# Meryx/ComputeRayTracer

Measured on AMD Instinct MI355X. Metric: Mrays/sec (+ HBM GB/s vs peak), 1080p 250k-tri scene, 1/2/4/8 MI355X, higher is better.
Workload: dtype f32; 1 GPU; S2 atrium250k: 253952 triangles + cornell walls/light, 1920x1080, 64 spp per step (BASELINE config 3)

## Files before the change

computeraytracer_amd/csrc/crt_device.h:

```cpp
#pragma once
#include <hip/hip_runtime.h>
#include <stdint.h>

namespace crt {

constexpr uint32_t kNoHit = 0xFFFFFFFFu;
constexpr int kStackDepth = 64;
constexpr uint32_t kNLambda = 301;
constexpr uint32_t kNCie = 471;
constexpr int CRT_NCOUNTERS_DEV = 16;

struct DevScene {
    const float4 *prim;
    const float4 *primD;
    const uint32_t *slot_of_index;
    const float4 *nodes;
    const float4 *nodes4;
    const uint4 *nodes4q;
    const uint4 *nodes8q;
    const float *spectra;
    const float *cie;
    const float4 *lights;
    uint32_t nprim;
    uint32_t npatch;
    int32_t root;
    int32_t root4;
    int32_t root8;
    uint32_t n_nodes4;
    uint32_t nspectra;
    uint32_t nlight;
    float hit_pad;
    uint32_t nf_last[2];
    float inv_nlight;
    uint32_t W, H;
    float qbase[3], qscale[3];
    float cam[12];
};

struct TraceParams {
    DevScene sc;
    uint32_t x0, y0, tw, th;
    uint32_t band, stride, phase;
    uint32_t first_sample, n_samples;
    float4 *accum;
    uchar4 *rgba;
    unsigned long long *counters;
    uint32_t tiles_x, tiles_y;
};

struct AsTiles {
    const uint32_t *active;
    const uint32_t *base;
    float *q;
    uint32_t n_active;
};

struct AsParams {
    const float4 *accum;
    const float *q;
    const uint32_t *counts;
    float *errors;
    uint32_t *flags;
    uint32_t *active;
    uint32_t *n_active;
    uint32_t tw, th, tiles_x, tiles_y;
    uint32_t min_samples, max_samples;
    float threshold;
};


constexpr uint32_t kWfAlive = 1u, kWfDying = 2u, kWfShadow = 4u, kWfSpecular = 8u, kWfInTrans = 16u;
constexpr uint32_t kWfNanRay = 1u << 31;
constexpr uint32_t kWfHasRad = 1u << 30;
constexpr uint32_t kWfListSlot = 0x7FFFFFFFu, kWfListAlsoExt = 0x80000000u;
constexpr uint32_t kWfDepthShift = 8, kWfLambdaShift = 16;
constexpr uint32_t kWfBatchShift = 25;
constexpr uint32_t kWfRing = 32;
constexpr uint32_t kWfSideCap = 65536;
constexpr uint32_t kWfOverflowLevels = 96;

constexpr uint32_t kWfShards = 64;
struct WfShard { uint32_t n[4], cur, n_dead, pad0[26], alive[kWfRing]; };
static_assert(sizeof(WfShard) == 256, "two lines per shard: the list counters and cursor, the per-batch counts");
struct WfWork { uint32_t cur, pad[31]; };
struct WfCtl {
    WfShard shard[4][kWfShards];
    unsigned long long counters[kWfShards][CRT_NCOUNTERS_DEV];
    uint32_t side_count[kWfRing];
    uint32_t dropped;
};
struct WfWorkQ {
    WfWork work[kWfShards];
    uint32_t work_done;
    uint32_t work_per_shard;
    unsigned long long work_total;
    uint32_t pad_[28];
};
static_assert(sizeof(WfWorkQ) == (kWfShards + 1) * 128, "whole lines");
struct WfSeg {
    unsigned long long work_total;
    uint32_t work_per_shard;
    uint32_t first_sample;
};

struct WfStatus {
    uint32_t it_end;
    uint32_t dropped;
    uint32_t bound;
    uint32_t pad_;
    unsigned long long rays;
    unsigned long long consumed[kWfRing];
    uint32_t left[kWfRing];
    uint32_t alive[kWfRing];
};

constexpr uint32_t kWfFinishSegs = 32;
struct WfFinishSegs {
    struct WfCtl *ctl[kWfFinishSegs];
    uint32_t base[kWfFinishSegs], batch[kWfFinishSegs];
    uint32_t n, blocks_per_seg;
};

struct WfParams {
    DevScene sc;
    float4 *ray_o, *ray_d, *sh_d, *beta, *radiance, *nee;
    uint4 *rng, *misc;
    float2 *hit;
    uint32_t *vis;
    float4 *recA, *recB;
    uint4 *recC;
    uint32_t *dead;
    uint32_t rearm;
    uint32_t gen_blocks;
    float4 *staging[kWfRing];
    uint32_t batch_id;
    WfStatus *status_out;
    uint32_t count_alive;
    uint32_t keep_pool;
    uint32_t side_base[kWfRing];
    uint32_t evict_mask;
    WfCtl *ctl;
    WfWorkQ *wq;
    WfSeg seg[kWfRing];
    uint32_t seg_order[kWfRing];
    uint32_t seg_n;
    uint32_t slot_base;
    uint32_t reset_wq;
    uint32_t P;
    uint32_t x0, y0, tw, th;
    uint32_t band, stride, phase;
    uint32_t tiles_x, tiles_y;
    uint32_t npix_padded;
    uint32_t list_cap;
    uint32_t tail_bound;
    uint32_t n_samples;
    float4 *accum;
    uchar4 *rgba;
    uchar4 *frames;
    uint32_t frame_ring;
    const uint32_t *tea;
    uint32_t count;
    uint32_t trace_form;
    int *stack_overflow;
    uint32_t overflow_lanes;
};

}
```

computeraytracer_amd/csrc/crt_wavefront.hip:

```cpp
#include "crt_shade.h"
#include <algorithm>

namespace crt {

#ifndef CRT_WF_STACK
#define CRT_WF_STACK 32
#endif
#ifndef CRT_WF_REFILL
#define CRT_WF_REFILL 24
#endif
#ifndef CRT_WF_INNER_RUN
#define CRT_WF_INNER_RUN 6
#endif
#ifndef CRT_WF_BURSTS
#define CRT_WF_BURSTS 4
#endif
#ifndef CRT_WF_BVH4
#define CRT_WF_BVH4 1
#endif
#ifndef CRT_WF_LEAF_AT
#define CRT_WF_LEAF_AT 32
#endif
#ifndef CRT_WF_SPEC
#define CRT_WF_SPEC 1
#endif
#ifndef CRT_WF_PATCH_RECOMPUTE
#define CRT_WF_PATCH_RECOMPUTE 20
#endif
#ifndef CRT_WF_SHADE_BLOCK
#define CRT_WF_SHADE_BLOCK 64
#endif
#ifndef CRT_WF_SHADE_MIN_WAVES
#define CRT_WF_SHADE_MIN_WAVES 1
#endif
#ifndef CRT_WF_MIN_WAVES
#define CRT_WF_MIN_WAVES 1
#endif
constexpr int kWfStack = CRT_WF_STACK;
constexpr int kNoNode = 0x7FFFFFFF;
constexpr int kTraceChunk = 128;
constexpr int kRefillAt = CRT_WF_REFILL;

__device__ __forceinline__ uint32_t lane_id() { return threadIdx.x & 63u; }

#ifndef CRT_WF_NT
#define CRT_WF_NT 1
#endif
typedef float v4f __attribute__((ext_vector_type(4)));
typedef float v2f __attribute__((ext_vector_type(2)));
typedef uint32_t v4u __attribute__((ext_vector_type(4)));
#if CRT_WF_NT
__device__ __forceinline__ float4 ldnt(const float4 *p) { const v4f v = __builtin_nontemporal_load((const v4f *)p); return float4{v.x, v.y, v.z, v.w}; }
__device__ __forceinline__ uint4 ldnt(const uint4 *p) { const v4u v = __builtin_nontemporal_load((const v4u *)p); return uint4{v.x, v.y, v.z, v.w}; }
__device__ __forceinline__ float2 ldnt(const float2 *p) { const v2f v = __builtin_nontemporal_load((const v2f *)p); return float2{v.x, v.y}; }
__device__ __forceinline__ uint32_t ldnt(const uint32_t *p) { return __builtin_nontemporal_load(p); }
__device__ __forceinline__ void stnt(float4 *p, float4 v) { __builtin_nontemporal_store(v4f{v.x, v.y, v.z, v.w}, (v4f *)p); }
__device__ __forceinline__ void stnt(uint4 *p, uint4 v) { __builtin_nontemporal_store(v4u{v.x, v.y, v.z, v.w}, (v4u *)p); }
__device__ __forceinline__ void stnt(float2 *p, float2 v) { __builtin_nontemporal_store(v2f{v.x, v.y}, (v2f *)p); }
__device__ __forceinline__ void stnt(uint32_t *p, uint32_t v) { __builtin_nontemporal_store(v, p); }
typedef uint32_t v2u __attribute__((ext_vector_type(2)));
__device__ __forceinline__ void stnt(uint2 *p, uint2 v) { __builtin_nontemporal_store(v2u{v.x, v.y}, (v2u *)p); }
#else
template <class T> __device__ __forceinline__ T ldnt(const T *p) { return *p; }
template <class T> __device__ __forceinline__ void stnt(T *p, T v) { *p = v; }
#endif
__device__ __forceinline__ uint32_t prefix_popc(unsigned long long mask, uint32_t lane)
{
    return (uint32_t)__popcll(mask & ((1ull << lane) - 1ull));
}

__device__ __noinline__ float2 resolve_nonfinite(const float4 *prim, const float4 *primD, const uint32_t *slot_of_index,
                                                 uint32_t nprim, float hit_pad, float ox, float oy, float oz, float dx,
                                                 float dy, float dz, uint32_t exclude)
{
    DevScene S{};
    S.prim = prim; S.primD = primD; S.slot_of_index = slot_of_index; S.nprim = nprim; S.hit_pad = hit_pad;
    float tm = CRT_INFINITY;
    uint32_t bi = kNoHit, bs = kNoHit;
    const f3 o = f3{ox, oy, oz}, d = f3{dx, dy, dz};
    for (uint32_t i = 0; i < nprim; i++) hit_test<true>(S, slot_of_index[i], o, d, exclude, 0.001f, tm, bi, bs);
    return float2{tm, bits_f(bs)};
}

struct PathRegs {
    f3 ray_o, ray_d;
    f4 beta, radiance;
    Rng rng;
    float last_pdf, etaScale;
    uint32_t exclude, work, flags;
};

__device__ __forceinline__ void wavelengths_of(uint32_t lambda, uint32_t wl[4])
{
    wl[0] = lambda; wl[1] = (lambda + 4u) % kNLambda; wl[2] = (lambda + 8u) % kNLambda;
    wl[3] = (lambda + 12u) % kNLambda;
}

struct LightRec { float4 L0, L1, L2, A, B, C, D; uint32_t slot; float pdf_area; };

template <bool UNIFORM>
__device__ __forceinline__ LightRec load_light(const DevScene &S, uint32_t li)
{
    LightRec r;
    r.A = float4{0.0f, 0.0f, 0.0f, 0.0f}; r.B = r.A; r.C = r.A; r.D = r.A; r.slot = kNoHit; r.pdf_area = 0.0f;
    if (UNIFORM) {
        typedef const __attribute__((address_space(4))) v4f *cptr4;
        typedef const __attribute__((address_space(4))) uint32_t *cptr1;
        auto ld = [](cptr4 p) { const v4f v = *p; return float4{v.x, v.y, v.z, v.w}; };
        const cptr4 lg = (cptr4)S.lights;
        r.L0 = ld(lg); r.L1 = ld(lg + 1); r.L2 = ld(lg + 2);
        const uint32_t include = f_bits(r.L1.w);
        if (include < S.nprim) {
            r.slot = ((cptr1)S.slot_of_index)[include];
            const cptr4 pg = (cptr4)S.prim + 3 * (size_t)r.slot;
            r.A = ld(pg); r.B = ld(pg + 1); r.C = ld(pg + 2); r.D = ld((cptr4)S.primD + r.slot);
            r.pdf_area = r.L2.w;
        }
    } else {
        r.L0 = S.lights[3 * li + 0]; r.L1 = S.lights[3 * li + 1]; r.L2 = S.lights[3 * li + 2];
        const uint32_t include = f_bits(r.L1.w);
        if (include < S.nprim) {
            r.slot = S.slot_of_index[include];
            r.A = S.prim[3 * (size_t)r.slot + 0]; r.B = S.prim[3 * (size_t)r.slot + 1]; r.C = S.prim[3 * (size_t)r.slot + 2];
            r.D = S.primD[r.slot];
            uint32_t l2 = (f_bits(r.A.w) >> 4) & 0x3FFFu;
            if (l2 >= S.nlight) l2 = S.nlight - 1u;
            r.pdf_area = S.lights[3 * l2 + 2].w;
        }
    }
    return r;
}

__device__ __forceinline__ f4 nee_term(const DevScene &S, const LightRec &L, f3 pos, f3 ldir, float t_l, float cos_theta,
                                       const f4 spec)
{
    f3 lp, ln; uint32_t lmeta;
    hit_attributes_rec(L.A, L.B, L.C, L.D, pos, ldir, t_l, lp, ln, lmeta);
    f4 le = spec * cos_theta;
    float pdf_l = compute_light_pdf_area(L.pdf_area, S.inv_nlight, lp, ln, pos, ldir);
    float pdf_b = cos_theta / CRT_PI;
    float weight_l = power_heuristic(1.0f, pdf_l, 1.0f, pdf_b);
    return (le * weight_l) / pdf_l;
}

struct ShadeCnt { uint32_t rays = 0, bounces = 0, shadow = 0, hits = 0, paths = 0, prims = 0, walk = 0; };
struct ShadowOut { bool emit; f3 d; float t_l; uint32_t l_index, l_slot; };

template <bool COUNT, bool FINISH>
__device__ __forceinline__ ShadowOut light_sample(const WfParams &P, const LightRec &L, uint32_t slot, f3 pos, f3 nrm, uint32_t b_index,
                                                  float u, float v2, f4 brdf, f4 beta, f4 &radiance, bool &rad_dirty, const uint32_t wl[4], ShadeCnt &cn)
{
    const DevScene &S = P.sc;
    ShadowOut out{false, f3{0.0f, 0.0f, 0.0f}, 0.0f, 0u, 0u};
    f3 pl = (xyz(L.L0) + xyz(L.L1) * u) + xyz(L.L2) * v2;
    f3 ldir = normalize(pl - pos);
    const uint32_t include = f_bits(L.L1.w);
    if (COUNT) { cn.rays++; cn.shadow++; }
    float t_l = CRT_INFINITY;
    uint32_t l_index = kNoHit, l_slot = kNoHit;
    const bool sh_finite = finite3(ldir) && finite3(pos);
    if (include < S.nprim && sh_finite) {
        hit_test_rec<false>(L.A, L.B, L.C, L.D, S.hit_pad, L.slot, pos, ldir, b_index, 0.001f, t_l, l_index, l_slot);
        if (COUNT) cn.prims++;
    }
    const float cos_theta = max_(0.0f, dot(nrm, ldir));
    if (!sh_finite) {
        const uint32_t w = S.nf_last[0] != b_index ? S.nf_last[0] : S.nf_last[1];
        if (COUNT) cn.prims += S.nprim;
        if (w != kNoHit && w == include) {
            if (COUNT) cn.hits++;
            const float qn = bits_f(0x7FC00000u);
            radiance = radiance + f4{qn, qn, qn, qn};
            rad_dirty = true;
        }
    } else if (l_slot != kNoHit && cos_theta > 0.0f) {
        if (COUNT) cn.hits++;
        const f4 nee = nee_term(S, L, pos, ldir, t_l, cos_theta, sample_spectrum(S, f_bits(L.L0.w), wl));
        f4 c = (brdf * nee) * beta;
#ifndef CRT_WHATIF_NO_NEE
        stnt(&P.nee[slot], float4{c.x, c.y, c.z, c.w});
#else
        if (c.x == 12345.678f) stnt(&P.nee[slot], float4{c.x, c.y, c.z, c.w});
#endif
        if (FINISH) {
            P.sh_d[slot] = float4{ldir.x, ldir.y, ldir.z, t_l};
            P.vis[slot] = include;
        }
        out = ShadowOut{true, ldir, t_l, include, l_slot};
        if (COUNT) cn.walk++;
    }
    return out;
}

struct ShadeOut {
    bool alive, emit_ext, emit_sh, sh_primary, rad_dirty; uint32_t batch;
    PathRegs R;
    f3 sd; float t_l; uint32_t l_index, l_slot;
};

#ifdef CRT_WF_PROBE
#define CRT_PROBE(tp, k) if (tp) { asm volatile("s_waitcnt vmcnt(0) lgkmcnt(0)" ::: "memory"); (tp)[k] = __builtin_readcyclecounter(); }
#else
#define CRT_PROBE(tp, k)
#endif

template <bool COUNT, bool FINISH>
__device__ __forceinline__ ShadeOut shade_body(const WfParams &P, uint32_t slot, bool in_pool, ShadeCnt &cn, unsigned long long *tp = nullptr)
{
    const DevScene &S = P.sc;
    PathRegs R;
    R.flags = 0;
    LightRec LU{};
    if (S.nlight == 1u) LU = load_light<true>(S, 0u);
    uint4 misc = uint4{0, 0, 0, 0}, rs = uint4{0, 0, 0, 0};
    float4 v_ro = float4{0, 0, 0, 0}, v_rd = v_ro, v_beta = v_ro, v_rad = v_ro, v_nee = v_ro;
    float2 h = float2{0.0f, 0.0f};
    uint32_t vis_in = 0;
    if (in_pool) {
        misc = ldnt(&P.misc[slot]); v_ro = ldnt(&P.ray_o[slot]); v_rd = ldnt(&P.ray_d[slot]); v_beta = ldnt(&P.beta[slot]);
        v_rad = ldnt(&P.radiance[slot]); rs = ldnt(&P.rng[slot]); h = ldnt(&P.hit[slot]); vis_in = ldnt(&P.vis[slot]);
#ifndef CRT_WHATIF_NO_NEE
        v_nee = ldnt(&P.nee[slot]);
#endif
    }
    CRT_PROBE(tp, 1)
    R.work = misc.x; R.flags = misc.y; R.last_pdf = bits_f(misc.z); R.etaScale = bits_f(misc.w);
    bool alive = in_pool && (R.flags & kWfAlive);
    bool emit_ext = false, emit_sh = false;
    bool sh_primary = false;
    bool finished = false, rad_dirty = false;
    f3 out_sd = f3{0, 0, 0}; float out_tl = 0.0f; uint32_t out_lindex = 0, out_lslot = 0;
    const bool nan_ray = alive && (R.flags & kWfNanRay) != 0u;
    if (nan_ray) R.flags &= ~kWfNanRay;
    const uint32_t h_slot = f_bits(h.y);
    const bool has_hit = alive && !nan_ray && !(R.flags & kWfDying) && h_slot != kNoHit;
    float4 hA = float4{0, 0, 0, 0}, hB = hA, hC = hA, hD = hA;
    if (has_hit) { hA = S.prim[3 * (size_t)h_slot + 0]; hB = S.prim[3 * (size_t)h_slot + 1]; hC = S.prim[3 * (size_t)h_slot + 2]; if (S.npatch) hD = S.primD[h_slot]; }
    CRT_PROBE(tp, 2)

    if (alive) {
        R.ray_o = xyz(v_ro); R.exclude = f_bits(v_ro.w);
        R.ray_d = xyz(v_rd);
        R.beta = f4{v_beta.x, v_beta.y, v_beta.z, v_beta.w};
        R.radiance = (R.flags & kWfHasRad) ? f4{v_rad.x, v_rad.y, v_rad.z, v_rad.w} : f4{0.0f, 0.0f, 0.0f, 0.0f};
        R.rng = Rng{rs.x, rs.y, rs.z, rs.w};
        uint32_t wl[4];
        wavelengths_of((R.flags >> kWfLambdaShift) & 0x1FFu, wl);
        uint32_t depth = (R.flags >> kWfDepthShift) & 0xFFu;

        if (R.flags & kWfShadow) {
            if (vis_in == 1u) { R.radiance = R.radiance + f4{v_nee.x, v_nee.y, v_nee.z, v_nee.w}; rad_dirty = true; }
            R.flags &= ~kWfShadow;
        }
        if (R.flags & kWfDying) {
            finished = true;
        } else if (nan_ray) {
            emit_ext = true;
        } else {
            const uint32_t b_slot = h_slot;
            if (COUNT) cn.bounces++;
            if (b_slot == kNoHit) {
                finished = true;
            } else {
                f3 pos, nrm;
                const f3 o = R.ray_o, d = R.ray_d;
                const uint32_t meta = f_bits(hA.w);
                pos = ray_at(o, d, h.x);
                if ((meta & 3u) == 1u) {
                    nrm = normalize(pos - xyz(hA));
                } else {
                    const f3 n0 = ((meta & 3u) == 0u) ? xyz(hD) : normalize(cross(xyz(hB), xyz(hC)));
                    nrm = (dot(n0, d) > 0.0f) ? -n0 : n0;
                }
                if (COUNT) cn.hits++;
                const uint32_t b_index = f_bits(hB.w);
                R.exclude = b_index;
                const uint32_t material = (meta >> 2) & 3u;
                const uint32_t emission_index = (meta >> 4) & 0x3FFFu;
                const uint32_t reflectance_index = (meta >> 18) & 0x3FFFu;
                if (material == kLight) {
                    f4 le = sample_spectrum(S, emission_index, wl);
                    if (depth == 0 || (R.flags & kWfSpecular)) {
                        R.radiance = R.radiance + R.beta * le;
                    } else {
                        float pdf_l = compute_light_pdf(S, emission_index, pos, nrm, o, d);
                        float weight_b = power_heuristic(1.0f, R.last_pdf, 1.0f, pdf_l);
                        R.radiance = R.radiance + (le * weight_b) * R.beta;
                    }
                    finished = true;
                } else if (depth >= kMaxDepthPath) {
                    finished = true;
                } else {
                    if (R.flags & kWfInTrans) {
                        float distance = length(o - pos);
                        f4 ext = sample_spectrum(S, S.nspectra - 1u, wl);
                        f4 att = f4{exp_(-ext.x * distance), exp_(-ext.y * distance), exp_(-ext.z * distance),
                                    exp_(-ext.w * distance)};
                        R.beta = R.beta * att;
                    }
                    if (material == kDiffuse) {
                        f4 brdf = sample_spectrum(S, reflectance_index, wl) / CRT_PI;
                        float u0 = rnd(R.rng);
                        uint32_t li = (uint32_t)((float)S.nlight * u0);
                        if (li >= S.nlight) li = S.nlight - 1u;
                        float u = rnd(R.rng);
                        float v2 = rnd(R.rng);
                        ShadowOut sh;
                        if (S.nlight == 1u) sh = light_sample<COUNT, FINISH>(P, LU, slot, pos, nrm, b_index, u, v2, brdf, R.beta, R.radiance, rad_dirty, wl, cn);
                        else sh = light_sample<COUNT, FINISH>(P, load_light<false>(S, li), slot, pos, nrm, b_index, u, v2, brdf, R.beta, R.radiance, rad_dirty, wl, cn);
                        if (sh.emit) {
                            emit_sh = true;
                            sh_primary = depth == 0u;
                            R.flags |= kWfShadow;
                            out_sd = sh.d; out_tl = sh.t_l; out_lindex = sh.l_index; out_lslot = sh.l_slot;
                        }
                        f3 new_direction = cosine_hemisphere(R.rng, nrm, R.last_pdf);
                        float cos_theta2 = abs_(dot(nrm, new_direction));
                        R.beta = R.beta * ((brdf * cos_theta2) / R.last_pdf);
                        R.ray_o = pos;
                        R.ray_d = new_direction;
                        R.flags &= ~kWfSpecular;
                    } else if (material == kGlass) {
                        const float eta1 = 1.0f, eta2 = 1.5f;
                        float eta = eta1 / eta2;
                        float cos_theta = dot(nrm, d);
                        float reflected = fresnel_s(d, nrm, eta1, eta2);
                        float pr = reflected;
                        float pt = 1.0f - reflected;
                        float u = rnd(R.rng);
                        f3 current_normal = nrm;
                        if (cos_theta > 0.0f) { eta = 1.0f / eta; current_normal = -current_normal; }
                        f3 new_direction;
                        if (u < pr / (pr + pt)) {
                            new_direction = reflect_(d, current_normal);
                        } else {
                            new_direction = normalize(refract_(d, current_normal, eta));
                            R.beta = R.beta * (eta * eta);
                            R.etaScale = R.etaScale / (eta * eta);
                            R.flags ^= kWfInTrans;
                        }
                        R.ray_o = pos;
                        R.flags |= kWfSpecular;
                        R.exclude = 0xFFFFFFFFu;
                        R.ray_d = new_direction;
                    }
                    bool rr_break = false;
                    {
                        f4 rbeta = R.beta * R.etaScale;
                        float max_beta_component = max_(rbeta.x, max_(rbeta.y, rbeta.z));
                        if (depth > 1u && max_beta_component < 1.0f) {
                            float qq = max_(0.0f, 1.0f - max_beta_component);
                            if (rnd(R.rng) < qq) rr_break = true;
                            else R.beta = R.beta / (1.0f - qq);
                        }
                    }
                    if (rr_break) {
                        if (emit_sh) R.flags |= kWfDying;
                        else finished = true;
                    } else {
                        depth++;
                        R.flags = (R.flags & ~(0xFFu << kWfDepthShift)) | (depth << kWfDepthShift);
                        emit_ext = true;
                        if (COUNT) { cn.rays++; cn.walk++; }
                    }
                }
            }
        }
        if (finished) {
            const uint32_t sample_off = R.work / P.npix_padded, pp = R.work % P.npix_padded;
            const uint32_t tile = pp >> 6, l = pp & 63u;
            const uint32_t lx = (tile % P.tiles_x) * 8u + (l & 7u), ly = (tile / P.tiles_x) * 8u + (l >> 3);
            f3 c = spectral_to_xyz(S, R.radiance, wl);
            stnt(&P.staging[(R.flags >> kWfBatchShift) & (kWfRing - 1u)][(size_t)sample_off * ((size_t)P.tw * P.th) + (size_t)ly * P.tw + lx], float4{c.x, c.y, c.z, 0.0f});
            alive = false;
            if (COUNT) cn.paths++;
        }
    }

    CRT_PROBE(tp, 3)
    if (!alive) R.flags = 0;
    ShadeOut so;
    so.alive = alive; so.emit_ext = emit_ext; so.emit_sh = emit_sh; so.sh_primary = sh_primary; so.rad_dirty = rad_dirty;
    so.batch = (R.flags >> kWfBatchShift) & (kWfRing - 1u);
    so.R = R; so.sd = out_sd; so.t_l = out_tl; so.l_index = out_lindex; so.l_slot = out_lslot;
    return so;
}

template <bool COUNT, bool FINISH>
__device__ __forceinline__ uint32_t shade_store(const WfParams &P, uint32_t slot, bool in_pool, ShadeOut &so, ShadeCnt &cn)
{
    const DevScene &S = P.sc;
    PathRegs &R = so.R;
    uint32_t resolved = 0u;
    if (in_pool) {
        const float4 vo = so.alive ? float4{R.ray_o.x, R.ray_o.y, R.ray_o.z, bits_f(R.exclude)} : float4{S.cam[9], S.cam[10], S.cam[11], bits_f(0xFFFFFFFFu)};
        stnt(&P.ray_o[slot], vo);
        if (so.alive) {
            if (so.emit_ext && (!finite3(R.ray_o) || !finite3(R.ray_d))) {
                P.hit[slot] = resolve_nonfinite(S.prim, S.primD, S.slot_of_index, S.nprim, S.hit_pad, R.ray_o.x, R.ray_o.y, R.ray_o.z,
                                                R.ray_d.x, R.ray_d.y, R.ray_d.z, R.exclude);
                if (COUNT) cn.prims += S.nprim;
                resolved = 1u;
            }
            stnt(&P.ray_d[slot], float4{R.ray_d.x, R.ray_d.y, R.ray_d.z, bits_f(resolved)});
            if (so.rad_dirty || (FINISH && !(R.flags & kWfHasRad))) {
                stnt(&P.radiance[slot], float4{R.radiance.x, R.radiance.y, R.radiance.z, R.radiance.w});
                R.flags |= kWfHasRad;
            }
            stnt(&P.rng[slot], uint4{R.rng.x, R.rng.y, R.rng.z, R.rng.w});
#ifdef CRT_WHATIF_EXTRA_STREAM
            if (!FINISH) { const float4 x = ldnt(&P.sh_d[slot]); stnt(&P.sh_d[slot], float4{x.y, x.x, x.w, x.z}); }
#endif
        }
        stnt(&P.beta[slot], so.alive ? float4{R.beta.x, R.beta.y, R.beta.z, R.beta.w} : float4{1.0f, 1.0f, 1.0f, 1.0f});
        stnt(&P.misc[slot], so.alive ? uint4{R.work, R.flags, f_bits(R.last_pdf), f_bits(R.etaScale)} : uint4{0u, 0u, f_bits(1.0f), f_bits(1.0f)});
    }
    return resolved;
}

__device__ __noinline__ void write_status(const WfCtl *ctl, const WfWorkQ *wq, uint32_t it_end, WfStatus *out)
{
    const uint32_t lane = lane_id();
    const WfShard &sh = ctl->shard[(it_end - 1u) & 3u][lane];
    const uint32_t mine = sh.n[0] + sh.n[1] + sh.n[2] + sh.n[3];
    unsigned long long rays = mine;
    uint32_t bound = mine;
    for (int off = 32; off > 0; off >>= 1) {
        rays += __shfl_xor(rays, off, 64);
        bound = max(bound, (uint32_t)__shfl_xor((int)bound, off, 64));
    }
    if (lane == 0) { out->dropped = ctl->dropped; out->bound = bound; out->pad_ = 0; out->rays = rays; }
#pragma unroll 1
    for (uint32_t g = 0; g < kWfRing; g += 8u) {
        unsigned long long cur[8];
        uint32_t alive[8];
#pragma unroll
        for (uint32_t k = 0; k < 8u; k++) {
            cur[k] = __hip_atomic_load(&wq[g + k].work[lane].cur, __ATOMIC_RELAXED, __HIP_MEMORY_SCOPE_AGENT);
            alive[k] = sh.alive[g + k];
        }
#pragma unroll
        for (uint32_t k = 0; k < 8u; k++) {
            const uint32_t b = g + k;
            const uint32_t wps = wq[b].work_per_shard;
            const unsigned long long wtot = wq[b].work_total, lo = (unsigned long long)lane * wps;
            const unsigned long long size = lo < wtot ? min((unsigned long long)wps, wtot - lo) : 0ull;
            unsigned long long cons = min(cur[k], size);
            const unsigned long long left = __ballot(cur[k] < size);
            uint32_t al = alive[k];
            for (int off = 32; off > 0; off >>= 1) {
                al += (uint32_t)__shfl_xor((int)al, off, 64);
                cons += __shfl_xor(cons, off, 64);
            }
            if (lane == 0) { out->alive[b] = al; out->consumed[b] = cons; out->left[b] = left ? 1u : 0u; }
        }
    }
    if (lane == 0) {
        __threadfence_system();
        __hip_atomic_store(&out->it_end, it_end, __ATOMIC_RELEASE, __HIP_MEMORY_SCOPE_SYSTEM);
    }
}

template <bool COUNT>
__global__ __launch_bounds__(CRT_WF_SHADE_BLOCK, CRT_WF_SHADE_MIN_WAVES) void k_wf_shade(const WfParams P, uint32_t it)
{
    const uint32_t ring = it & 3u, lbuf = it & 1u;
    WfCtl *ctl = P.ctl;
    static_assert(kWfShards == 64, "one lane per shard");
    if (blockIdx.x == 0 && threadIdx.x < 64u && P.status_out != nullptr) write_status(P.ctl, P.wq, it, P.status_out);
    if (blockIdx.x == 0 && threadIdx.x < kWfShards) {
        WfShard &nx = ctl->shard[(it + 1u) & 3u][threadIdx.x];
        nx.n[0] = 0; nx.n[1] = 0; nx.n[2] = 0; nx.n[3] = 0; nx.cur = 0; nx.n_dead = 0;
        for (uint32_t b = 0; b < kWfRing; b++) nx.alive[b] = 0;
    }
    uint32_t slot, my_shard;
    bool in_pool;
    if (P.tail_bound == 0u) {
        const uint32_t local = blockIdx.x * (uint32_t)CRT_WF_SHADE_BLOCK + threadIdx.x;
        slot = P.slot_base + local;
        my_shard = blockIdx.x % kWfShards;
        in_pool = local < P.P;
    } else {
        const uint32_t bps = (4u * P.tail_bound + (uint32_t)CRT_WF_SHADE_BLOCK - 1u) / (uint32_t)CRT_WF_SHADE_BLOCK;
        my_shard = blockIdx.x / bps;
        const uint32_t j = (blockIdx.x % bps) * (uint32_t)CRT_WF_SHADE_BLOCK + threadIdx.x;
        const WfShard &pv = ctl->shard[(it + 3u) & 3u][my_shard];
        const size_t region = (size_t)my_shard * P.list_cap;
        slot = 0; in_pool = false;
        const uint32_t cls = j / P.tail_bound, e = j % P.tail_bound;
        if (cls < 4u && e < pv.n[cls]) {
            const size_t g = (size_t)((lbuf ^ 1u) * 4u + cls) * ((size_t)P.list_cap * kWfShards) + region + e;
            const uint32_t entry = cls < 2u ? f_bits(ldnt(&P.recB[g]).w) : ldnt(&P.recC[g]).x;
            slot = entry & kWfListSlot;
            in_pool = cls < 2u || !(entry & kWfListAlsoExt);
        }
    }
    if (P.evict_mask) {
        uint4 misc = uint4{0, 0, 0, 0};
        if (in_pool) misc = P.misc[slot];
        const uint32_t par = (misc.y >> kWfBatchShift) & (kWfRing - 1u);
        const bool go = in_pool && (misc.y & kWfAlive) && ((P.evict_mask >> par) & 1u);
        for (uint32_t b = 0; b < kWfRing; b++) {
            if (!((P.evict_mask >> b) & 1u)) continue;
            const unsigned long long m = __ballot(go && par == b);
            if (!m) continue;
            uint32_t base = 0;
            if (lane_id() == 0) base = atomicAdd(&ctl->side_count[b], (uint32_t)__popcll(m));
            base = __shfl(base, 0, 64);
            const uint32_t idx = base + prefix_popc(m, lane_id());
            if (go && par == b && idx >= kWfSideCap) atomicAdd(&ctl->dropped, 1u);
            if (go && par == b && idx < kWfSideCap) {
                const uint32_t d = P.side_base[b] + idx;
                P.ray_o[d] = P.ray_o[slot]; P.ray_d[d] = P.ray_d[slot]; P.sh_d[d] = P.sh_d[slot]; P.beta[d] = P.beta[slot];
                P.radiance[d] = P.radiance[slot]; P.nee[d] = P.nee[slot]; P.rng[d] = P.rng[slot]; P.hit[d] = P.hit[slot];
                P.vis[d] = P.vis[slot]; P.misc[d] = misc;
                P.misc[slot] = uint4{0, 0, 0, 0};
            }
        }
    }
    ShadeCnt cn;
#ifdef CRT_WF_PROBE
    unsigned long long tpa[8];
    unsigned long long *tp = (!COUNT && P.tail_bound == 0u && (blockIdx.x & 255u) == 7u) ? tpa : nullptr;
    tpa[0] = __builtin_readcyclecounter();
#else
    unsigned long long *tp = nullptr;
#endif
    ShadeOut so = shade_body<COUNT, false>(P, slot, in_pool, cn, tp);
    CRT_PROBE(tp, 4)
    const bool emit_ext = so.emit_ext, emit_sh = so.emit_sh, sh_primary = so.sh_primary;
    {
        const uint32_t lane = lane_id();
        const bool cl2 = emit_sh && sh_primary, cl3 = emit_sh && !sh_primary;
        const bool dead = in_pool && !so.alive && P.rearm != 0u;
        const unsigned long long m1 = __ballot(emit_ext), m2 = __ballot(cl2), m3 = __ballot(cl3), md = __ballot(dead);
        WfShard &sh = ctl->shard[ring][my_shard];
        uint32_t b1 = 0, b2 = 0, b3 = 0, bd = 0;
        if (lane == 0) {
            if (m1) b1 = atomicAdd(&sh.n[1], (uint32_t)__popcll(m1));
            if (m2) b2 = atomicAdd(&sh.n[2], (uint32_t)__popcll(m2));
            if (m3) b3 = atomicAdd(&sh.n[3], (uint32_t)__popcll(m3));
            if (md) bd = atomicAdd(&sh.n_dead, (uint32_t)__popcll(md));
        }
        if (P.count_alive) {
            unsigned long long am = __ballot(so.alive);
            while (am) {
                const uint32_t b = (uint32_t)__shfl((int)so.batch, __ffsll((long long)am) - 1, 64);
                const unsigned long long m = __ballot(so.alive && so.batch == b);
                if (lane == 0) atomicAdd(&sh.alive[b], (uint32_t)__popcll(m));
                am &= ~m;
            }
        }
        const uint32_t resolved = shade_store<COUNT, false>(P, slot, in_pool, so, cn);
        CRT_PROBE(tp, 5)
        b1 = __shfl(b1, 0, 64); b2 = __shfl(b2, 0, 64); b3 = __shfl(b3, 0, 64); bd = __shfl(bd, 0, 64);
        const size_t region = (size_t)my_shard * P.list_cap;
        const size_t cls_stride = (size_t)P.list_cap * kWfShards;
        const PathRegs &R = so.R;
        if (emit_ext) {
            const size_t g = (size_t)(lbuf * 4u + 1u) * cls_stride + region + b1 + prefix_popc(m1, lane);
            stnt(&P.recA[g], float4{R.ray_o.x, R.ray_o.y, R.ray_o.z, bits_f(R.exclude)});
            stnt(&P.recB[g], float4{R.ray_d.x, R.ray_d.y, R.ray_d.z, bits_f(slot | (resolved ? kWfListAlsoExt : 0u))});
        }
        if (emit_sh) {
            const uint32_t c = cl2 ? 2u : 3u;
            const size_t g = (size_t)(lbuf * 4u + c) * cls_stride + region + (cl2 ? b2 + prefix_popc(m2, lane) : b3 + prefix_popc(m3, lane));
            stnt(&P.recA[g], float4{R.ray_o.x, R.ray_o.y, R.ray_o.z, bits_f(R.exclude)});
            stnt(&P.recB[g], float4{so.sd.x, so.sd.y, so.sd.z, so.t_l});
            stnt(&P.recC[g], uint4{slot | (emit_ext ? kWfListAlsoExt : 0u), so.l_index, so.l_slot, 0u});
        }
        if (dead) stnt(&P.dead[region + bd + prefix_popc(md, lane)], slot);
    }
    if (COUNT) {
        wave_add(ctl->counters[blockIdx.x % kWfShards] + CRT_CNT_RAYS, cn.rays);
        wave_add(ctl->counters[blockIdx.x % kWfShards] + CRT_CNT_BOUNCES, cn.bounces);
        wave_add(ctl->counters[blockIdx.x % kWfShards] + CRT_CNT_SHADOW, cn.shadow);
        wave_add(ctl->counters[blockIdx.x % kWfShards] + CRT_CNT_HITS, cn.hits);
        wave_add(ctl->counters[blockIdx.x % kWfShards] + CRT_CNT_PATHS, cn.paths);
        wave_add(ctl->counters[blockIdx.x % kWfShards] + CRT_CNT_PRIMS, cn.prims);
        wave_add(ctl->counters[blockIdx.x % kWfShards] + CRT_CNT_WALKED, cn.walk);
    }
#ifdef CRT_WF_PROBE
    CRT_PROBE(tp, 6)
    if (tp && lane_id() == 0) {
        for (int k = 0; k < 6; k++) atomicAdd(ctl->counters[blockIdx.x % kWfShards] + 8 + k, tp[k + 1] - tp[k]);
        atomicAdd(ctl->counters[blockIdx.x % kWfShards] + 14, 1ull);
    }
#endif
}

__device__ __forceinline__ uint32_t wf_as_tile(const AsTiles &A, uint32_t w)
{
    return A.active[(w % (A.n_active * 64u)) >> 6];
}

template <bool COUNT, bool ADAPT>
__global__ __launch_bounds__(64) void k_wf_gen(const WfParams P, uint32_t it, const AsTiles A)
{
    const DevScene &S = P.sc;
    const uint32_t ring = it & 3u, lbuf = it & 1u;
    WfCtl *ctl = P.ctl;
    const uint32_t lane = lane_id();
    const uint32_t my_shard = blockIdx.x % kWfShards, j = blockIdx.x / kWfShards;
    WfShard &sh = ctl->shard[ring][my_shard];
    const uint32_t n_chunks = min(sh.n_dead, P.list_cap) / 64u;
    if (j >= n_chunks) return;
    const uint32_t mine = (n_chunks - j + P.gen_blocks - 1u) / P.gen_blocks;
    const size_t region = (size_t)my_shard * P.list_cap;
    const size_t cls_stride = (size_t)P.list_cap * kWfShards;
    uint32_t seg_q[2] = {0, 0}, seg_n[2] = {0, 0}, nseg = 0, want = mine;
    uint32_t seg_w[2] = {0, 0};
    for (uint32_t si = 0; si < P.seg_n && want > 0u && nseg < 2u; si++) {
        const uint32_t sg = P.seg_order[si];
        WfWorkQ *wq = P.wq + sg;
        const uint32_t wps = P.seg[sg].work_per_shard;
        const unsigned long long wtot = P.seg[sg].work_total, lo = (unsigned long long)my_shard * wps;
        const uint32_t size = lo < wtot ? (uint32_t)min((unsigned long long)wps, wtot - lo) : 0u;
        if (__hip_atomic_load(&wq->work[my_shard].cur, __ATOMIC_RELAXED, __HIP_MEMORY_SCOPE_AGENT) >= size) continue;
        uint32_t base = 0;
        if (lane == 0) base = atomicAdd(&wq->work[my_shard].cur, want * 64u);
        base = (uint32_t)__builtin_amdgcn_readfirstlane((int)base);
        if (base >= size) continue;
        const uint32_t got = min(want, (size - base) / 64u);
        seg_q[nseg] = sg; seg_w[nseg] = (uint32_t)lo + base; seg_n[nseg] = got; nseg++;
        want -= got;
    }
    for (uint32_t si = 0; si < P.seg_n && nseg == 0u; si++) {
        const uint32_t sg = P.seg_order[si];
        WfWorkQ *wq = P.wq + sg;
        if (__hip_atomic_load(&wq->work_done, __ATOMIC_RELAXED, __HIP_MEMORY_SCOPE_AGENT) != 0u) continue;
        const uint32_t wps = P.seg[sg].work_per_shard;
        const unsigned long long wtot = P.seg[sg].work_total, lo_l = (unsigned long long)lane * wps;
        const uint32_t size_l = lo_l < wtot ? (uint32_t)min((unsigned long long)wps, wtot - lo_l) : 0u;
        const uint32_t cur_l = __hip_atomic_load(&wq->work[lane].cur, __ATOMIC_RELAXED, __HIP_MEMORY_SCOPE_AGENT);
        const unsigned long long avail = __ballot(cur_l < size_l);
        if (!avail) {
            if (lane == 0) __hip_atomic_store(&wq->work_done, 1u, __ATOMIC_RELAXED, __HIP_MEMORY_SCOPE_AGENT);
            continue;
        }
        const uint32_t rot = my_shard & 63u;
        const unsigned long long rmask = rot ? ((avail >> rot) | (avail << (64u - rot))) : avail;
        const uint32_t s_pick = ((uint32_t)(__ffsll((long long)rmask) - 1) + rot) & 63u;
        uint32_t base = 0;
        if (lane == 0) base = atomicAdd(&wq->work[s_pick].cur, want * 64u);
        base = (uint32_t)__builtin_amdgcn_readfirstlane((int)base);
        const uint32_t size_s = (uint32_t)__shfl((int)size_l, (int)s_pick, 64);
        if (base >= size_s) continue;
        const uint32_t got = min(want, (size_s - base) / 64u);
        seg_q[0] = sg; seg_w[0] = s_pick * wps + base; seg_n[0] = got; nseg = 1;
        want -= got;
    }
    const uint32_t total = seg_n[0] + seg_n[1];
    if (total == 0u) return;
    const bool ragged = ((P.tw | P.th) & 7u) != 0u;
    uint32_t n_valid[2] = {seg_n[0] * 64u, seg_n[1] * 64u};
    if (ragged) {
        for (uint32_t g = 0; g < 2u; g++) {
            n_valid[g] = 0;
            for (uint32_t k = 0; k < seg_n[g]; k++) {
                const uint32_t tile = ADAPT ? wf_as_tile(A, seg_w[g] + 64u * k) : ((seg_w[g] + 64u * k) % P.npix_padded) >> 6;
                const uint32_t lx = (tile % P.tiles_x) * 8u + (lane & 7u), ly = (tile / P.tiles_x) * 8u + (lane >> 3);
                n_valid[g] += (uint32_t)__popcll(__ballot(lx < P.tw && ly < P.th));
            }
        }
    }
    uint32_t b0 = 0;
    if (lane == 0) {
        b0 = atomicAdd(&sh.n[0], n_valid[0] + n_valid[1]);
        if (P.count_alive) {
            if (n_valid[0]) atomicAdd(&sh.alive[seg_q[0]], n_valid[0]);
            if (n_valid[1]) atomicAdd(&sh.alive[seg_q[1]], n_valid[1]);
        }
    }
    uint32_t c_rays = 0, pos = 0;
    bool have_b0 = false;
    for (uint32_t k = 0; k < total; k++) {
        const uint32_t g = k < seg_n[0] ? 0u : 1u, kk = g ? k - seg_n[0] : k;
        const uint32_t sg = seg_q[g];
        const uint32_t w0 = seg_w[g] + 64u * kk;
        uint32_t sample_off = w0 / P.npix_padded, pp0 = w0 % P.npix_padded;
        if (ADAPT) {
            sample_off = w0 / (A.n_active * 64u);
            pp0 = wf_as_tile(A, w0) * 64u;
        }
        const uint32_t tile = pp0 >> 6;
        const uint32_t lx = (tile % P.tiles_x) * 8u + (lane & 7u), ly = (tile / P.tiles_x) * 8u + (lane >> 3);
        const bool valid = lx < P.tw && ly < P.th;
        const unsigned long long mv = __ballot(valid);
        const uint32_t slot = ldnt(&P.dead[region + (size_t)(j + k * P.gen_blocks) * 64u + lane]);
        f3 eye = f3{0.0f, 0.0f, 0.0f}, d = eye;
        uint32_t resolved = 0u;
        if (valid) {
            const uint32_t px = P.x0 + lx, sample = ADAPT ? A.base[tile] + P.seg[sg].first_sample + sample_off : P.seg[sg].first_sample + sample_off;
            const uint32_t py = P.y0 + (ly / P.band) * P.band * P.stride + P.phase * P.band + ly % P.band;
            Rng rng = Rng{py, px * 100u, sample, P.tea[(size_t)ly * P.tw + lx]};
            const float jx = rnd(rng);
            const float fs = ((float)px + ((float)(sample % kGrid) + jx) / (float)kGrid) / (float)S.W;
            const float jy = rnd(rng);
            const float ft = ((float)S.H - (float)py + ((float)(sample % kGrid) + jy) / (float)kGrid) / (float)S.H;
            const f3 llc = f3{S.cam[0], S.cam[1], S.cam[2]}, hor = f3{S.cam[3], S.cam[4], S.cam[5]};
            const f3 ver = f3{S.cam[6], S.cam[7], S.cam[8]};
            eye = f3{S.cam[9], S.cam[10], S.cam[11]};
            d = normalize(((llc + hor * fs) + ver * ft) - eye);
            const float ul = rnd(rng);
            const uint32_t lambda = (uint32_t)(301.0f * ul);
            const bool nan_ray = !finite3(eye) || !finite3(d);
            const uint32_t flags = kWfAlive | (lambda << kWfLambdaShift) | (sg << kWfBatchShift) | (nan_ray ? kWfNanRay : 0u);
            stnt(&P.ray_d[slot], float4{d.x, d.y, d.z, bits_f(0u)});
            stnt(&P.rng[slot], uint4{rng.x, rng.y, rng.z, rng.w});
            stnt((uint2 *)&P.misc[slot], uint2{(ADAPT ? sample_off * P.npix_padded + pp0 : w0) + lane, flags});
            if (!finite3(eye) || !finite3(d)) resolved = 1u;
        }
        if (!have_b0) { b0 = (uint32_t)__builtin_amdgcn_readfirstlane((int)b0); have_b0 = true; }
        if (valid) {
            const size_t e = (size_t)(lbuf * 4u) * cls_stride + region + b0 + pos + prefix_popc(mv, lane);
            stnt(&P.recA[e], float4{eye.x, eye.y, eye.z, bits_f(0xFFFFFFFFu)});
            stnt(&P.recB[e], float4{d.x, d.y, d.z, bits_f(slot | (resolved ? kWfListAlsoExt : 0u))});
            if (COUNT) c_rays++;
        }
        pos += (uint32_t)__popcll(mv);
    }
    if (COUNT) {
        wave_add(ctl->counters[blockIdx.x % kWfShards] + CRT_CNT_RAYS, c_rays);
        wave_add(ctl->counters[blockIdx.x % kWfShards] + CRT_CNT_WALKED, c_rays);
    }
}

__device__ __forceinline__ void tri_test(const float4 A, const float4 B, const float4 C, uint32_t slot, f3 o, f3 d,
                                         uint32_t exclude, float t_min, float hit_pad, float &t_max,
                                         uint32_t &b_index, uint32_t &b_slot)
{
    const uint32_t index = f_bits(B.w);
    const f3 v0 = xyz(A), e1 = xyz(B), e2 = xyz(C);
    const f3 pvec = cross(d, e2);
    const float det = dot(e1, pvec);
    const float inv = 1.0f / det;
    const f3 tvec = o - v0;
    const float u = dot(tvec, pvec) * inv;
    const f3 qvec = cross(tvec, e1);
    const float v = dot(d, qvec) * inv;
    const float t = dot(e2, qvec) * inv;
    const bool ok = (exclude != index) & (det != 0.0f) & (u >= 0.0f) & (u <= 1.0f) & (v >= 0.0f) & ((u + v) <= 1.0f) &
                    beats<false>(t, t_min, t_max, index, b_index, b_slot);
    if (ok) {
        const f3 p = ray_at(o, d, t);
        const f3 v1 = v0 + e1, v2 = v0 + e2;
        const bool in = p.x >= min_(v0.x, min_(v1.x, v2.x)) - hit_pad && p.x <= max_(v0.x, max_(v1.x, v2.x)) + hit_pad &&
                        p.y >= min_(v0.y, min_(v1.y, v2.y)) - hit_pad && p.y <= max_(v0.y, max_(v1.y, v2.y)) + hit_pad &&
                        p.z >= min_(v0.z, min_(v1.z, v2.z)) - hit_pad && p.z <= max_(v0.z, max_(v1.z, v2.z)) + hit_pad;
        if (in) { t_max = t; b_index = index; b_slot = slot; }
    }
}

__device__ __forceinline__ int stack_pop(const int *stk, const int *ovf, size_t ovl, int sp)
{
    int v = stk[(sp < kWfStack ? sp : kWfStack - 1) * 64];
    if (sp >= kWfStack) v = *(const volatile int *)(ovf + (size_t)(sp - kWfStack) * ovl);
    return v;
}

template <bool COUNT, int QUANT>
__global__ __launch_bounds__(64, CRT_WF_MIN_WAVES) void k_wf_trace(const WfParams P, uint32_t it)
{
    __shared__ int lds_stack[kWfStack * 64];
    WfCtl *ctl = P.ctl;
    const float4 *__restrict__ nodes = CRT_WF_BVH4 ? P.sc.nodes4 : P.sc.nodes;
    const uint4 *__restrict__ nodesq = QUANT == 2 ? P.sc.nodes8q : P.sc.nodes4q;
    const f3 qscale = f3{P.sc.qscale[0], P.sc.qscale[1], P.sc.qscale[2]}, qbase = f3{P.sc.qbase[0], P.sc.qbase[1], P.sc.qbase[2]};
    const float4 *__restrict__ prim = P.sc.prim;
    const float4 *__restrict__ primD = P.sc.primD;
    uint32_t *__restrict__ g_vis = P.vis;
    float2 *__restrict__ g_hit = P.hit;
    const size_t cls_stride = (size_t)P.list_cap * kWfShards;
    const float4 *__restrict__ recA = P.recA + (size_t)((it & 1u) * 4u) * cls_stride;
    const float4 *__restrict__ recB = P.recB + (size_t)((it & 1u) * 4u) * cls_stride;
    const uint4 *__restrict__ recC = P.recC + (size_t)((it & 1u) * 4u) * cls_stride;
    const float hit_pad = P.sc.hit_pad;
    const int root = QUANT == 2 ? P.sc.root8 : CRT_WF_BVH4 ? P.sc.root4 : P.sc.root;
    int *__restrict__ ovf = P.stack_overflow + ((size_t)blockIdx.x * 64 + lane_id());
    const size_t ovl = P.overflow_lanes;
    const uint32_t nprim = P.sc.nprim;
    DevScene S = P.sc;
    S.prim = prim; S.primD = primD;

    const uint32_t ring = it & 3u;
    const uint32_t lane = lane_id();
    int *stk = lds_stack + lane;
    const float t_min = 0.001f;

    uint32_t cur_shard = blockIdx.x % kWfShards, sh_e0 = 0, sh_e1 = 0, sh_e2 = 0, sh_total = 0;
    uint32_t chunk_pos = 0, chunk_end = 0;
    bool have_shard = false, exhausted = false;
    {
        const WfShard &so = ctl->shard[ring][cur_shard];
        sh_e0 = so.n[0]; sh_e1 = sh_e0 + so.n[1]; sh_e2 = sh_e1 + so.n[2]; sh_total = sh_e2 + so.n[3];
        have_shard = sh_total > 0u;
    }
    bool active = false;
    int pend = 0;
    f3 o = f3{0, 0, 0}, d = f3{0, 0, 0}, id = f3{0, 0, 0}, oid = f3{0, 0, 0};
    uint32_t excl = 0, slot = 0, b_index = kNoHit, b_slot = kNoHit, b_slot_in = kNoHit;
    float t_max = 0.0f;
    bool shadow = false;
    int node = 0, sp = 0;
    int nx = 0, ny = 0, nz = 0;
    uint32_t c_nodes = 0, c_prims = 0;
    uint32_t d_inner_it = 0, d_inner_act = 0, d_leaf_it = 0, d_leaf_act = 0, d_prim_it = 0, d_refill = 0, d_refill_lanes = 0, d_scans = 0;

    for (;;) {
        const unsigned long long idle = __ballot(!active);
        const int nidle = __popcll(idle);
        if (!exhausted && nidle >= kRefillAt) {
            for (int guard = 0; chunk_pos == chunk_end && !exhausted && guard < 2 * (int)kWfShards; guard++) {
                if (have_shard) {
                    uint32_t base = 0;
                    if (lane == 0) base = atomicAdd(&ctl->shard[ring][cur_shard].cur, (uint32_t)kTraceChunk);
                    base = __shfl(base, 0, 64);
                    if (base < sh_total) { chunk_pos = base; chunk_end = min(base + (uint32_t)kTraceChunk, sh_total); break; }
                    have_shard = false;
                }
                if (COUNT) d_scans++;
                const WfShard &sl = ctl->shard[ring][lane % kWfShards];
                const uint32_t e0 = sl.n[0], e1 = e0 + sl.n[1], e2 = e1 + sl.n[2], tot = e2 + sl.n[3];
                const uint32_t cur_l = __hip_atomic_load(&sl.cur, __ATOMIC_RELAXED, __HIP_MEMORY_SCOPE_AGENT);
                const unsigned long long avail = __ballot(cur_l < tot);
                if (!avail) { exhausted = true; break; }
                const uint32_t rot = cur_shard & 63u;
                const unsigned long long rmask = rot ? ((avail >> rot) | (avail << (64u - rot))) : avail;
                cur_shard = ((uint32_t)(__ffsll((long long)rmask) - 1) + rot) & 63u;
                sh_e0 = __shfl(e0, (int)cur_shard, 64); sh_e1 = __shfl(e1, (int)cur_shard, 64);
                sh_e2 = __shfl(e2, (int)cur_shard, 64); sh_total = __shfl(tot, (int)cur_shard, 64);
                have_shard = true;
            }
            if (chunk_pos < chunk_end) {
                const uint32_t give = min((uint32_t)nidle, chunk_end - chunk_pos);
                if (COUNT) { d_refill++; d_refill_lanes += give; }
                const uint32_t my = prefix_popc(idle, lane);
                if (!active && my < give) {
                    const uint32_t idx = chunk_pos + my;
                    const size_t region = (size_t)cur_shard * P.list_cap;
                    shadow = idx >= sh_e1;
                    const size_t g = idx < sh_e0 ? region + idx : idx < sh_e1 ? cls_stride + region + (idx - sh_e0)
                                   : idx < sh_e2 ? 2u * cls_stride + region + (idx - sh_e1) : 3u * cls_stride + region + (idx - sh_e2);
                    const float4 ro = ldnt(&recA[g]), rd = ldnt(&recB[g]);
                    uint4 rc = uint4{0, 0, 0, 0};
                    if (shadow) rc = ldnt(&recC[g]);
                    o = xyz(ro); excl = f_bits(ro.w);
                    d = xyz(rd);
                    active = true;
                    if (shadow) {
                        slot = rc.x & kWfListSlot; t_max = rd.w;
                        b_index = rc.y;
                        b_slot = rc.z;
                    } else {
                        slot = f_bits(rd.w) & kWfListSlot;
                        t_max = CRT_INFINITY; b_index = kNoHit; b_slot = kNoHit;
                        if (f_bits(rd.w) & kWfListAlsoExt) active = false;
                        else if (nprim == 0u) { g_hit[slot] = float2{t_max, bits_f(kNoHit)}; active = false; }
                    }
                    b_slot_in = b_slot;
                    node = root; sp = 0; pend = 0;
                    const float tiny = 1.0e-20f;
                    id.x = 1.0f / (abs_(d.x) > tiny ? d.x : __builtin_copysignf(tiny, d.x));
                    id.y = 1.0f / (abs_(d.y) > tiny ? d.y : __builtin_copysignf(tiny, d.y));
// ... 810 lines not shown
```

Baseline: 7310 Mrays/s.

## Regenerate fresh camera rays in shade instead of storing ray_d, rng, beta

Ray generation now writes only a misc record carrying the sample index and seed plus a new kFresh flag, and no longer stores ray_d and rng. The shade kernel recomputes the camera ray, RNG state, beta and pdf for fresh paths from the pixel and seed. Dead slots no longer write ray_o or beta defaults. The aim is to cut HBM write and read traffic per new path, at the cost of extra ALU work in shade. It relies on work_pixel reproducing the pixel mapping, and the misc.z/w fields are reused for sample and seed. In the ADAPT case the work index encodes pp0 rather than the raw w0, so that reconstruction may not be exact there.

```diff
diff --git a/computeraytracer_amd/csrc/crt_device.h b/computeraytracer_amd/csrc/crt_device.h
--- a/computeraytracer_amd/csrc/crt_device.h
+++ b/computeraytracer_amd/csrc/crt_device.h
@@ -70,6 +70,7 @@
 
 
 constexpr uint32_t kWfAlive = 1u, kWfDying = 2u, kWfShadow = 4u, kWfSpecular = 8u, kWfInTrans = 16u;
+constexpr uint32_t kWfFresh = 32u;
 constexpr uint32_t kWfNanRay = 1u << 31;
 constexpr uint32_t kWfHasRad = 1u << 30;
 constexpr uint32_t kWfListSlot = 0x7FFFFFFFu, kWfListAlsoExt = 0x80000000u;
diff --git a/computeraytracer_amd/csrc/crt_wavefront.hip b/computeraytracer_amd/csrc/crt_wavefront.hip
--- a/computeraytracer_amd/csrc/crt_wavefront.hip
+++ b/computeraytracer_amd/csrc/crt_wavefront.hip
@@ -82,6 +82,34 @@
     return float2{tm, bits_f(bs)};
 }
 
+struct CamRay { f3 eye, d; Rng rng; uint32_t lambda; bool nan_ray; };
+__device__ __forceinline__ CamRay camera_ray(const DevScene &S, uint32_t px, uint32_t py, uint32_t sample, uint32_t seed)
+{
+    CamRay c;
+    c.rng = Rng{py, px * 100u, sample, seed};
+    const float jx = rnd(c.rng);
+    const float fs = ((float)px + ((float)(sample % kGrid) + jx) / (float)kGrid) / (float)S.W;
+    const float jy = rnd(c.rng);
+    const float ft = ((float)S.H - (float)py + ((float)(sample % kGrid) + jy) / (float)kGrid) / (float)S.H;
+    const f3 llc = f3{S.cam[0], S.cam[1], S.cam[2]}, hor = f3{S.cam[3], S.cam[4], S.cam[5]};
+    const f3 ver = f3{S.cam[6], S.cam[7], S.cam[8]};
+    c.eye = f3{S.cam[9], S.cam[10], S.cam[11]};
+    c.d = normalize(((llc + hor * fs) + ver * ft) - c.eye);
+    const float ul = rnd(c.rng);
+    c.lambda = (uint32_t)(301.0f * ul);
+    c.nan_ray = !finite3(c.eye) || !finite3(c.d);
+    return c;
+}
+
+__device__ __forceinline__ void work_pixel(const WfParams &P, uint32_t work, uint32_t &px, uint32_t &py)
+{
+    const uint32_t pp = work % P.npix_padded;
+    const uint32_t tile = pp >> 6, l = pp & 63u;
+    const uint32_t lx = (tile % P.tiles_x) * 8u + (l & 7u), ly = (tile / P.tiles_x) * 8u + (l >> 3);
+    px = P.x0 + lx;
+    py = P.y0 + (ly / P.band) * P.band * P.stride + P.phase * P.band + ly % P.band;
+}
+
 struct PathRegs {
     f3 ray_o, ray_d;
     f4 beta, radiance;
@@ -239,11 +267,22 @@
     CRT_PROBE(tp, 2)
 
     if (alive) {
+        if (R.flags & kWfFresh) {
+            uint32_t px, py;
+            work_pixel(P, R.work, px, py);
+            const CamRay c = camera_ray(S, px, py, misc.z, misc.w);
+            v_ro = float4{c.eye.x, c.eye.y, c.eye.z, bits_f(0xFFFFFFFFu)};
+            v_rd = float4{c.d.x, c.d.y, c.d.z, 0.0f};
+            v_beta = float4{1.0f, 1.0f, 1.0f, 1.0f};
+            rs = uint4{c.rng.x, c.rng.y, c.rng.z, c.rng.w};
+            R.last_pdf = 1.0f; R.etaScale = 1.0f;
+            R.flags &= ~kWfFresh;
+        }
         R.ray_o = xyz(v_ro); R.exclude = f_bits(v_ro.w);
         R.ray_d = xyz(v_rd);
         R.beta = f4{v_beta.x, v_beta.y, v_beta.z, v_beta.w};
+        R.rng = Rng{rs.x, rs.y, rs.z, rs.w};
         R.radiance = (R.flags & kWfHasRad) ? f4{v_rad.x, v_rad.y, v_rad.z, v_rad.w} : f4{0.0f, 0.0f, 0.0f, 0.0f};
-        R.rng = Rng{rs.x, rs.y, rs.z, rs.w};
         uint32_t wl[4];
         wavelengths_of((R.flags >> kWfLambdaShift) & 0x1FFu, wl);
         uint32_t depth = (R.flags >> kWfDepthShift) & 0xFFu;
@@ -393,9 +432,8 @@
     PathRegs &R = so.R;
     uint32_t resolved = 0u;
     if (in_pool) {
-        const float4 vo = so.alive ? float4{R.ray_o.x, R.ray_o.y, R.ray_o.z, bits_f(R.exclude)} : float4{S.cam[9], S.cam[10], S.cam[11], bits_f(0xFFFFFFFFu)};
-        stnt(&P.ray_o[slot], vo);
         if (so.alive) {
+            stnt(&P.ray_o[slot], float4{R.ray_o.x, R.ray_o.y, R.ray_o.z, bits_f(R.exclude)});
             if (so.emit_ext && (!finite3(R.ray_o) || !finite3(R.ray_d))) {
                 P.hit[slot] = resolve_nonfinite(S.prim, S.primD, S.slot_of_index, S.nprim, S.hit_pad, R.ray_o.x, R.ray_o.y, R.ray_o.z,
                                                 R.ray_d.x, R.ray_d.y, R.ray_d.z, R.exclude);
@@ -411,9 +449,9 @@
 #ifdef CRT_WHATIF_EXTRA_STREAM
             if (!FINISH) { const float4 x = ldnt(&P.sh_d[slot]); stnt(&P.sh_d[slot], float4{x.y, x.x, x.w, x.z}); }
 #endif
-        }
-        stnt(&P.beta[slot], so.alive ? float4{R.beta.x, R.beta.y, R.beta.z, R.beta.w} : float4{1.0f, 1.0f, 1.0f, 1.0f});
-        stnt(&P.misc[slot], so.alive ? uint4{R.work, R.flags, f_bits(R.last_pdf), f_bits(R.etaScale)} : uint4{0u, 0u, f_bits(1.0f), f_bits(1.0f)});
+            stnt(&P.beta[slot], float4{R.beta.x, R.beta.y, R.beta.z, R.beta.w});
+        }
+        stnt(&P.misc[slot], so.alive ? uint4{R.work, R.flags, f_bits(R.last_pdf), f_bits(R.etaScale)} : uint4{0u, 0u, 0u, 0u});
     }
     return resolved;
 }
@@ -693,23 +731,12 @@
         if (valid) {
             const uint32_t px = P.x0 + lx, sample = ADAPT ? A.base[tile] + P.seg[sg].first_sample + sample_off : P.seg[sg].first_sample + sample_off;
             const uint32_t py = P.y0 + (ly / P.band) * P.band * P.stride + P.phase * P.band + ly % P.band;
-            Rng rng = Rng{py, px * 100u, sample, P.tea[(size_t)ly * P.tw + lx]};
-            const float jx = rnd(rng);
-            const float fs = ((float)px + ((float)(sample % kGrid) + jx) / (float)kGrid) / (float)S.W;
-            const float jy = rnd(rng);
-            const float ft = ((float)S.H - (float)py + ((float)(sample % kGrid) + jy) / (float)kGrid) / (float)S.H;
-            const f3 llc = f3{S.cam[0], S.cam[1], S.cam[2]}, hor = f3{S.cam[3], S.cam[4], S.cam[5]};
-            const f3 ver = f3{S.cam[6], S.cam[7], S.cam[8]};
-            eye = f3{S.cam[9], S.cam[10], S.cam[11]};
-            d = normalize(((llc + hor * fs) + ver * ft) - eye);
-            const float ul = rnd(rng);
-            const uint32_t lambda = (uint32_t)(301.0f * ul);
-            const bool nan_ray = !finite3(eye) || !finite3(d);
-            const uint32_t flags = kWfAlive | (lambda << kWfLambdaShift) | (sg << kWfBatchShift) | (nan_ray ? kWfNanRay : 0u);
-            stnt(&P.ray_d[slot], float4{d.x, d.y, d.z, bits_f(0u)});
-            stnt(&P.rng[slot], uint4{rng.x, rng.y, rng.z, rng.w});
-            stnt((uint2 *)&P.misc[slot], uint2{(ADAPT ? sample_off * P.npix_padded + pp0 : w0) + lane, flags});
-            if (!finite3(eye) || !finite3(d)) resolved = 1u;
+            const uint32_t seed = P.tea[(size_t)ly * P.tw + lx];
+            const CamRay c = camera_ray(S, px, py, sample, seed);
+            eye = c.eye; d = c.d;
+            const uint32_t flags = kWfAlive | kWfFresh | (c.lambda << kWfLambdaShift) | (sg << kWfBatchShift) | (c.nan_ray ? kWfNanRay : 0u);
+            stnt(&P.misc[slot], uint4{(ADAPT ? sample_off * P.npix_padded + pp0 : w0) + lane, flags, sample, seed});
+            if (c.nan_ray) resolved = 1u;
         }
         if (!have_b0) { b0 = (uint32_t)__builtin_amdgcn_readfirstlane((int)b0); have_b0 = true; }
         if (valid) {
```

After: 7419 Mrays/s (median of 6 runs). +1.5%, better.
